# aweisberg/cassandra-accord

Measured on AMD Instinct MI355X. Metric: txn-key conflict pairs resolved/sec (node), higher is better.
Workload: dtype u32/u64 (integer); 1 GPU; config2: KeyDeps batch, 1M txns x 8 keys, zipf(0.99) over 1M keys, p_write 0.5, uncommitted window 10k, per-GPU CommandStore snapshot; key_distribution=zipf, keys_permuted=True, n_txn_per_gpu=1000000, pairs_per_gpu=8000000, dep_edges_per_gpu=35349420, parallelism=keyspace shards x1 (independent CommandStores)

## Files before the change

### cassandra-accord_amd/accord_amd/_lib.py

```python
from __future__ import annotations

import ctypes as C
import os

HERE = os.path.dirname(os.path.abspath(__file__))
LIB_PATH = os.environ.get("ACC_LIB_PATH") or os.path.join(HERE, "libaccord_amd.so")

ACC_OK, ACC_E_ARG, ACC_E_STATE, ACC_E_NOMEM, ACC_E_DEVICE, ACC_E_CAP = 0, -1, -2, -3, -4, -5
ACC_MEM_HOST, ACC_MEM_DEVICE = 0, 1
ACC_OPT_TIMING = 1
ACC_OPT_FORCE_REPLAY = 2
ACC_OPT_NO_WINDOW_TIER = 4
ACC_OPT_TIER_GRID_SHIFT = 16
ACC_OPT_RD_WIDE_SORT = 8
ACC_OPT_PD_SERIAL = 16
ACC_OPT_KD_NO_STREAM_AHEAD = 32
ACC_LV_AUTO, ACC_LV_LDS_WALK, ACC_LV_WINDOWED, ACC_LV_WAVES = 0, 1, 2, 3
ACC_STARTED_BEFORE, ACC_STARTED_AFTER, ACC_STARTED_ANY = 0, 1, 2
ACC_DEP_WITH, ACC_DEP_WITHOUT, ACC_DEP_ANY = 0, 1, 2
ACC_STATUS_ANY, ACC_STATUS_IS_PROPOSED, ACC_STATUS_IS_STABLE = 0, 1, 2
ACC_FULL_EXECUTES_AFTER = 1
ACC_LATEST_PROPOSAL, ACC_LATEST_COMMIT = 0, 1
RECOVERY_SCANS = {
    "acceptedOrCommittedStartedBeforeWithoutWitnessing": (ACC_STARTED_BEFORE, ACC_DEP_WITHOUT, ACC_STATUS_IS_PROPOSED, True),
# ... 11 lines not shown
           "acc_keydeps_batch", "acc_keydeps_copy_out", "acc_keydeps_mixed", "acc_rangedeps_batch", "acc_rangedeps_copy_out",
           "acc_shard_pack", "acc_shard_merge", "acc_keydeps_merge", "acc_merge_copy_out", "acc_levelise",
           "acc_timing_count", "acc_timing_get", "acc_timing_reset", "acc_timing_filter", "acc_stats_count", "acc_stats_get",
           "acc_deps_merge", "acc_rmm_copy_out", "acc_rmm_invert", "acc_rmm_slice", "acc_rangedeps_stab", "acc_copy_out", "acc_comm_unique_id", "acc_comm_init_rccl", "acc_comm_init_host", "acc_comm_destroy", "acc_partial_deps_reduce", "acc_shard_reduce",
           "acc_map_reduce_full", "acc_map_reduce_full_ranges", "acc_latest_deps_merge", "acc_partial_deps_batch",
           "acc_deps_from_json", "acc_deps_to_json",
           "acc_cfk_create", "acc_cfk_destroy", "acc_cfk_update", "acc_cfk_view", "acc_cfk_apply", "acc_cfk_snap_to_batch",
           "acc_cfk_apply_deps", "acc_cfk_state", "acc_cfk_missing", "acc_cfk_keydeps", "acc_cfk_keydeps_mixed",
           "acc_cfk_map_reduce_full", "acc_cfk_redundant_before", "acc_cfk_redundant_view", "acc_max_conflicts",
           "acc_maxconflicts_create", "acc_maxconflicts_destroy", "acc_maxconflicts_update", "acc_maxconflicts_get",
           "acc_maxconflicts_size",
           "acc_rcmd_create", "acc_rcmd_destroy", "acc_rcmd_update", "acc_rcmd_view", "acc_rcmd_rangedeps",
           "acc_rcmd_update_cmds", "acc_rcmd_state_view", "acc_rcmd_map_reduce_full",
           "acc_ranges_of", "acc_ranges_with", "acc_ranges_subtract", "acc_ranges_merge_touching", "acc_ranges_select",
           "acc_ranges_index_of", "acc_ranges_contains_all_keys", "acc_ranges_contains_all", "acc_rangedeps_is_covered_by",
           "acc_partial_deps_covering", "acc_rmm_without", "acc_recovery_deps_reduce"]


class Opts(C.Structure):
    _fields_ = [("flags", C.c_uint32), ("wave_grid_max", C.c_uint32), ("cfk_hot", C.c_uint32), ("lv_tier", C.c_uint32),
                ("lv_chunk", C.c_uint32), ("cfq_wave_cap", C.c_uint32)]


class TsCols(C.Structure):
    _fields_ = [("msb", C.c_void_p), ("lsb", C.c_void_p), ("node", C.c_void_p)]


class BatchIn(C.Structure):
    _fields_ = [("n_txn", C.c_uint32), ("mem", C.c_uint32), ("n_pairs", C.c_uint64),
                ("txn_id", TsCols), ("execute_at", TsCols),
                ("status", C.c_void_p), ("key_off", C.c_void_p), ("key_code", C.c_void_p)]
# ... 501 lines not shown
        L.acc_rcmd_view.argtypes = [C.c_void_p, C.c_void_p, C.POINTER(RcmdTable)]
        L.acc_rcmd_view.restype = C.c_int
        L.acc_rcmd_rangedeps.argtypes = [C.c_void_p, C.c_void_p, C.POINTER(CfkMixedQueries), C.POINTER(RangedepsView)]
        L.acc_rcmd_rangedeps.restype = C.c_int
        L.acc_rcmd_update_cmds.argtypes = [C.c_void_p, C.c_void_p, C.POINTER(RcmdCmdUpdates)]
        L.acc_rcmd_update_cmds.restype = C.c_int
        L.acc_rcmd_state_view.argtypes = [C.c_void_p, C.c_void_p, C.POINTER(RcmdState)]
        L.acc_rcmd_state_view.restype = C.c_int
        L.acc_rcmd_map_reduce_full.argtypes = [C.c_void_p, C.c_void_p, C.POINTER(CfkRecoveryIn), C.POINTER(RangedepsView)]
        L.acc_rcmd_map_reduce_full.restype = C.c_int
    except AttributeError:
        if not os.environ.get("ACC_LIB_PATH"):
            raise
    L.acc_copy_out.argtypes = [C.c_void_p, C.c_void_p, C.c_void_p, C.c_size_t, C.c_uint32]
    L.acc_copy_out.restype = C.c_int
    L.acc_timing_count.argtypes = [C.c_void_p]
    L.acc_timing_count.restype = C.c_int
    L.acc_timing_get.argtypes = [C.c_void_p, C.c_int, C.POINTER(C.c_char_p), C.POINTER(C.c_double),
                                 C.POINTER(C.c_uint64)]
    L.acc_timing_get.restype = C.c_int
    L.acc_timing_reset.argtypes = [C.c_void_p]
    L.acc_timing_reset.restype = None
    L.acc_timing_filter.argtypes = [C.c_void_p, C.c_char_p]
    L.acc_timing_filter.restype = C.c_int
    L.acc_stats_count.argtypes = [C.c_void_p]
    L.acc_stats_count.restype = C.c_int
    L.acc_stats_get.argtypes = [C.c_void_p, C.c_int, C.POINTER(C.c_char_p), C.POINTER(C.c_uint64)]
    L.acc_stats_get.restype = C.c_int
    _lib = L
    return L
# ... 1 lines not shown
```

### cassandra-accord_amd/accord_amd/deps.py

```python
from __future__ import annotations

import ctypes as C
from dataclasses import dataclass

import numpy as np

from . import _lib as L


class AccordError(RuntimeError):
    code = None


class IllegalArgumentException(AccordError):
    code = L.ACC_E_ARG


class IllegalStateException(AccordError):
    code = L.ACC_E_STATE


class DeviceError(AccordError):
    code = L.ACC_E_DEVICE

# ... 82 lines not shown

    def stats(self) -> dict:
        out = {}
        for i in range(max(self._lib.acc_stats_count(self._h), 0)):
            name = C.c_char_p()
            val = C.c_uint64()
            self._lib.acc_stats_get(self._h, i, C.byref(name), C.byref(val))
            out[name.value.decode()] = val.value
        return out

    def timing_reset(self):
        self._lib.acc_timing_reset(self._h)

    def timing_filter(self, tags=None):
        self.check(self._lib.acc_timing_filter(self._h, ",".join(tags).encode() if tags else None))

    def keydeps_batch_raw(self, batch_in: "L.BatchIn") -> "L.KeydepsView":
        view = L.KeydepsView()
        self.check(self._lib.acc_keydeps_batch(self._h, C.byref(batch_in), C.byref(view)))
        return view

    def calculate_partial_deps(self, batch) -> "BatchKeyDeps":
        arrs = dict(tm=np.ascontiguousarray(batch.txn_msb, dtype=np.uint64),
                    tl=np.ascontiguousarray(batch.txn_lsb, dtype=np.uint64),
                    tn=np.ascontiguousarray(batch.txn_node, dtype=np.int32),
                    em=np.ascontiguousarray(batch.exe_msb, dtype=np.uint64),
                    el=np.ascontiguousarray(batch.exe_lsb, dtype=np.uint64),
                    en=np.ascontiguousarray(batch.exe_node, dtype=np.int32),
                    st=np.ascontiguousarray(batch.status, dtype=np.uint8),
                    ko=np.ascontiguousarray(batch.key_off, dtype=np.uint32),
# ... 1146 lines not shown
```

### cassandra-accord_amd/csrc/api.hip

```cpp
#include "dict.hpp"
#include <exception>
#include <thread>

namespace acc {
void keydeps_batch(acc_ctx *ctx, const acc_batch_in *in, acc_keydeps_view *view);
void keydeps_mixed(acc_ctx *ctx, const acc_range_batch_in *in, acc_keydeps_view *view, SharedDict *shared = nullptr);
void keydeps_merge(acc_ctx *ctx, const acc_merge_in *in, acc_merge_view *view);
void levelise(acc_ctx *ctx, const acc_graph_in *in, uint32_t *level, uint32_t *order, uint32_t *n_levels);
void rangedeps_batch(acc_ctx *ctx, const acc_range_batch_in *in, acc_rangedeps_view *view, const SharedDict *shared = nullptr);
void shard_pack(acc_ctx *ctx, const acc_batch_in *in, acc_frag_streams *out, bool ctx_alloc);
void shard_merge(acc_ctx *ctx, const acc_frag_recv *in, acc_merge_view *view);
void deps_merge(acc_ctx *ctx, const acc_deps_merge_in *in, acc_deps_merge_view *view);
void rmm_invert(acc_ctx *ctx, const acc_rmm_batch *in, acc_csr_view *out);
void rmm_slice(acc_ctx *ctx, const acc_rmm_batch *in, const acc_ranges_in *select, acc_slice_view *out);
void rangedeps_stab(acc_ctx *ctx, const acc_rmm_batch *rd, const acc_stab_in *q, acc_stab_view *out);
void rmm_without(acc_ctx *ctx, const acc_rmm_batch *in, const acc_ts_cols *txn, const acc_txn_sets *set_a,
                 const acc_txn_sets *set_b, acc_without_view *out);
void recovery_deps_reduce(acc_ctx *ctx, const acc_deps_merge_in *cw, const acc_deps_merge_in *anw, acc_recovery_deps_view *view);
void map_reduce_full(acc_ctx *ctx, const acc_batch_in *in, const acc_recovery_in *q, acc_keydeps_view *view);
void map_reduce_full_ranges(acc_ctx *ctx, const acc_range_cmds_in *c, const acc_recovery_ranges_in *q, acc_rangedeps_view *view);
void latest_deps_merge(acc_ctx *ctx, const acc_latest_in *in, acc_latest_view *view);
void deps_from_json(acc_ctx *ctx, const acc_json_in *in, acc_json_deps_view *view);
void deps_to_json(acc_ctx *ctx, const acc_json_out_in *in, acc_json_out *out);
void cfk_update(acc_ctx *ctx, acc_cfk *cfk, const acc_batch_in *in);
// ... 93 lines not shown
}

}

extern "C" {

const char *acc_last_error(const acc_ctx *ctx) { return ctx ? ctx->last_error.c_str() : "null context"; }

int acc_sync(acc_ctx *ctx)
{
    if (!ctx) return ACC_E_ARG;
    return acc_guard(ctx, [&] { ctx->sync(); });
}

void *acc_stream(acc_ctx *ctx) { return ctx ? (void *)ctx->stream : nullptr; }

int acc_keydeps_batch(acc_ctx *ctx, const acc_batch_in *in, acc_keydeps_view *out_view)
{
    if (!ctx) return ACC_E_ARG;
    return acc_guard(ctx, [&] {
        ACC_HIP(hipSetDevice(ctx->device));
        acc::keydeps_batch(ctx, in, out_view);
    });
}

int acc_keydeps_mixed(acc_ctx *ctx, const acc_range_batch_in *in, acc_keydeps_view *out_view)
{
    if (!ctx) return ACC_E_ARG;
    return acc_guard(ctx, [&] {
        ACC_HIP(hipSetDevice(ctx->device));
// ... 612 lines not shown
```

### cassandra-accord_amd/csrc/keydeps.hip

```cpp
#include "keydeps.hpp"

#include <vector>

namespace acc {


struct TxnInfoArgs {
    uint32_t n = 0;
    const uint8_t *status = nullptr;
    const uint64_t *tl = nullptr;
    uint4 *tinfo = nullptr;
    uint32_t *bigflag = nullptr;
};

__device__ __forceinline__ void txn_info_one(uint32_t t, uint32_t n, const uint32_t *rank, const uint8_t *status,
                                             const uint64_t *tl, const uint32_t *key_off, uint4 *tinfo, uint32_t *bigflag)
{
    if (bigflag) bigflag[t] = 0;
    const uint32_t kind = (uint32_t)(tl[t] >> 1) & 7u;
    tinfo[t] = make_uint4(rank[t], rank[n + t], (uint32_t)status[t] | (kind << 3), key_off[t]);
}

__global__ __launch_bounds__(BLOCK) void k_pair_keys(size_t P, const uint64_t *__restrict__ key_code,
                                                     const uint32_t *__restrict__ owner, const uint32_t *__restrict__ key_off,
// ... 1 lines not shown
                                                     const uint32_t *__restrict__ perm, PairPlan plan,
                                                     int rank_only, uint64_t *__restrict__ out, TxnInfoArgs ti)
{
    size_t i = (size_t)blockIdx.x * BLOCK + threadIdx.x;
    if (ti.tinfo && i < ti.n) txn_info_one((uint32_t)i, ti.n, rank, ti.status, ti.tl, key_off, ti.tinfo, ti.bigflag);
    if (i >= P) return;
    size_t j = perm ? perm[i] : i;
    if (rank_only) { out[i] = rank[owner[j]]; return; }
    uint64_t kc = pext_runs(key_code[j], plan.rk);
    if (plan.mode == 4) {
        const uint32_t t = owner[j];
        out[i] = (kc << 32) | ((uint64_t)t << plan.sb) | (uint64_t)(j - key_off[t]);
        return;
    }
    out[i] = plan.mode == 1 ? ((kc << plan.rbits) | rank[owner[j]]) : plan.mode == 3 ? ((kc << 32) | i) : kc;
}

__global__ __launch_bounds__(BLOCK) void k_seg_flags_packed(size_t P, const uint64_t *__restrict__ sp, uint32_t *__restrict__ flag,
                                                            uint32_t *__restrict__ perm, int sb, const uint32_t *__restrict__ key_off,
                                                            uint32_t *__restrict__ pown)
{
    size_t p = (size_t)blockIdx.x * BLOCK + threadIdx.x;
    if (p >= P) return;
    const uint64_t x = sp[p];
    flag[p] = p == 0 || (x >> 32) != (sp[p - 1] >> 32);
    if (sb < 0) { perm[p] = (uint32_t)x; return; }
    const uint32_t t = (uint32_t)x >> sb, slot = (uint32_t)x & ((1u << sb) - 1u);
    perm[p] = key_off[t] + slot;
    pown[p] = t;
}
// ... 2413 lines not shown
    const size_t P = cb.P;
    const uint32_t *key_off = cb.key_off;
    const uint64_t *key_code = cb.key_code;
    const uint32_t *owner = cb.owner, *rank = cb.dict.rank;
    const int rbits = cb.dict.rbits;
    PairPlan &pp = cb.pp;
    uint64_t *pkey = ctx->get<uint64_t>("pair_key", P);
    const unsigned gP = grid_for(P, BLOCK);
    PairSort s;
    s.seg_flag = ctx->get<uint32_t>("seg_flag", P);
    if (cb.dict.batch_sorted && pp.rk.bits <= 32) {
        const bool m4 = bits_for((uint64_t)n - 1) + pp.sb <= 32;
        pp.mode = m4 ? 4 : 3;
        TxnInfoArgs ti;
        if (!keys_only) { ti.n = n; ti.status = cb.status; ti.tl = cb.tl; ti.tinfo = cb.tinfo; ti.bigflag = cb.bigflag; }
        launch(ctx, "pair_keys", k_pair_keys, dim3(grid_for(std::max<size_t>(P, n), BLOCK)), dim3(BLOCK), 0, P, key_code,
               owner, key_off, rank, (const uint32_t *)nullptr, pp, 0, pkey, ti);
        s.tinfo_done = !keys_only;
        const uint64_t *sp = radix_sort_keys(ctx, "rs_pair", pkey, P, 32, pp.rk.bits);
        uint32_t *perm = ctx->get<uint32_t>("pair_perm", P + V2_ITEMS);
        if (m4) s.sp_m4 = sp;
        else launch(ctx, "seg_flags", k_seg_flags_packed, dim3(gP), dim3(BLOCK), 0, P, sp, s.seg_flag, perm, -1, key_off,
                    (uint32_t *)nullptr);
        s.ps = { nullptr, perm };
        s.flags_done = true;
    } else if (cb.dict.batch_sorted) {
        pp.mode = 0;
        launch(ctx, "pair_keys", k_pair_keys, dim3(gP), dim3(BLOCK), 0, P, key_code, owner, key_off, rank,
               (const uint32_t *)nullptr, pp, 0, pkey, TxnInfoArgs{});
        s.ps = radix_sort(ctx, "rs_pair", pkey, nullptr, P, pp.rk.bits);
    } else if (pp.rk.bits + rbits <= 64) {
        pp.mode = 1;
        launch(ctx, "pair_keys", k_pair_keys, dim3(gP), dim3(BLOCK), 0, P, key_code, owner, key_off, rank,
               (const uint32_t *)nullptr, pp, 0, pkey, TxnInfoArgs{});
// ... 579 lines not shown
```

### cassandra-accord_amd/csrc/prims.hpp

```cpp
#pragma once

#include "ctx.hpp"

#include <algorithm>
#include <vector>

namespace acc {


__device__ __forceinline__ uint32_t lane_id() { return threadIdx.x & 63u; }

template <class T>
__device__ __forceinline__ T shfl_up(T v, unsigned d)
{
    if constexpr (sizeof(T) == 8) {
        uint64_t u = (uint64_t)v;
        uint32_t lo = __shfl_up((uint32_t)u, d, 64), hi = __shfl_up((uint32_t)(u >> 32), d, 64);
        return (T)(((uint64_t)hi << 32) | lo);
    } else {
        return (T)__shfl_up((uint32_t)v, d, 64);
    }
}

template <class T>
// ... 393 lines not shown

__device__ __forceinline__ uint64_t pext_runs(uint64_t w, const Runs &r)
{
    uint64_t o = 0;
    for (int i = 0; i < r.n; ++i) {
        uint64_t m = r.len[i] >= 64 ? ~0ull : ((1ull << r.len[i]) - 1);
        o |= ((w >> r.lo[i]) & m) << r.dst[i];
    }
    return o;
}


constexpr int RS_ITEMS = 16;
constexpr int RS_TILE = BLOCK * RS_ITEMS;
constexpr int RS_ITEMS_S = 4;
constexpr int RS_TILE_S = BLOCK * RS_ITEMS_S;
constexpr size_t rs_small_n() { return (size_t)256 << 10; }

static __global__ __launch_bounds__(BLOCK) void k_rs_hist(const uint64_t *__restrict__ keys, size_t n, int shift,
                                                   uint32_t *__restrict__ hist, uint32_t ntiles)
{
    __shared__ uint32_t h[256];
    h[threadIdx.x] = 0;
    __syncthreads();
    const size_t base = (size_t)blockIdx.x * RS_TILE;
#pragma unroll 4
    for (int k = 0; k < RS_ITEMS; ++k) {
        size_t e = base + (size_t)k * BLOCK + threadIdx.x;
        if (e < n) atomicAdd(&h[(keys[e] >> shift) & 255u], 1u);
    }
// ... 84 lines not shown
        }
    }
    __syncthreads();
    for (uint32_t i = tid; i < tile_total; i += BLOCK) {
        const uint64_t key = sk[i];
        const uint32_t d = (uint32_t)(key >> shift) & 255u;
        const uint32_t dst = gbase[d] + (i - lbase[d]);
        kout[dst] = key;
        vout[dst] = sv[i];
    }
}

constexpr uint32_t OS_AGG = 1u << 30, OS_INC = 2u << 30, OS_VAL = (1u << 30) - 1;
constexpr int OS_MAXP = 8;

static __global__ __launch_bounds__(BLOCK) void k_rs_ghist(const uint64_t *__restrict__ keys, size_t n, int lo, int passes,
                                                    uint32_t *__restrict__ ghist, uint32_t *__restrict__ other, uint32_t other_n)
{
    __shared__ uint32_t h[WAVES][OS_MAXP][256];
    const uint32_t tid = threadIdx.x, wave = tid >> 6, lane = lane_id();
    for (uint32_t i = blockIdx.x * BLOCK + tid; i < other_n; i += gridDim.x * BLOCK) other[i] = 0;
    for (uint32_t i = tid; i < WAVES * OS_MAXP * 256; i += BLOCK) (&h[0][0][0])[i] = 0;
    __syncthreads();
    for (size_t base = (size_t)blockIdx.x * RS_TILE; base < n; base += (size_t)gridDim.x * RS_TILE) {
    uint64_t key[RS_ITEMS];
#pragma unroll
    for (int k = 0; k < RS_ITEMS; ++k) {
        const size_t e = base + (size_t)k * BLOCK + tid;
        key[k] = e < n ? keys[e] : 0;
    }
    for (int p = 0; p < passes; ++p) {
#pragma unroll
        for (int k = 0; k < RS_ITEMS; ++k) {
            const bool valid = base + (size_t)k * BLOCK + tid < n;
            const uint32_t d = (uint32_t)(key[k] >> (lo + 8 * p)) & 255u;
            const uint32_t d0 = (uint32_t)__shfl((int)d, 0, 64);
            const uint64_t vb = __ballot(valid);
            if (__ballot(valid && d == d0) == vb) {
                if (lane == 0) h[wave][p][d0] += (uint32_t)__popcll(vb);
            } else if (valid) {
                atomicAdd(&h[wave][p][d], 1u);
            }
        }
    }
    }
    __syncthreads();
    for (uint32_t i = tid; i < (uint32_t)passes * 256; i += BLOCK) {
        uint32_t s = 0;
#pragma unroll
        for (int w = 0; w < WAVES; ++w) s += h[w][i >> 8][i & 255];
        if (s) atomicAdd(&ghist[i], s);
    }
}

__device__ __forceinline__ void os_store(uint32_t *p, uint32_t w) { __hip_atomic_store(p, w, __ATOMIC_RELAXED, __HIP_MEMORY_SCOPE_AGENT); }
__device__ __forceinline__ uint32_t os_load(const uint32_t *p) { return __hip_atomic_load(p, __ATOMIC_RELAXED, __HIP_MEMORY_SCOPE_AGENT); }

template <bool KO, int ITEMS>
static __global__ __launch_bounds__(BLOCK) void k_rs_onesweep(const uint64_t *__restrict__ kin, const uint32_t *__restrict__ vin,
                                                       uint64_t *__restrict__ kout, uint32_t *__restrict__ vout, size_t n,
                                                       int shift, const uint32_t *__restrict__ dtotal,
                                                       uint32_t *__restrict__ status, uint32_t *__restrict__ ticket,
                                                       int iota_vals)
{
    __shared__ uint64_t sk[(BLOCK * ITEMS)];
    __shared__ uint32_t sv[KO ? 1 : (BLOCK * ITEMS)];
    __shared__ uint32_t cnt[WAVES][256];
    __shared__ uint32_t wpre[WAVES][256];
    __shared__ uint32_t run[256], lbase[256], gbase[256];
    __shared__ uint32_t red[WAVES];
    __shared__ uint32_t s_b;
    const uint32_t tid = threadIdx.x, lane = lane_id(), wave = tid >> 6;
    const uint64_t lt_mask = (lane == 0) ? 0ull : ((~0ull) >> (64 - lane));
    if (tid == 0) s_b = atomicAdd(ticket, 1u);
    run[tid] = 0;
#pragma unroll
    for (int w = 0; w < WAVES; ++w) cnt[w][tid] = 0;
    __syncthreads();
    const uint32_t b = s_b;
    const size_t base = (size_t)b * (BLOCK * ITEMS);
    uint64_t key[ITEMS];
    uint32_t val[ITEMS], lr[ITEMS], pk[ITEMS];
#pragma unroll
    for (int k = 0; k < ITEMS; ++k) {
        const size_t e = base + (size_t)k * BLOCK + tid;
        const bool valid = e < n;
        key[k] = valid ? kin[e] : 0;
        if constexpr (!KO) val[k] = valid ? (iota_vals ? (uint32_t)e : vin[e]) : 0;
    }
#pragma unroll
    for (int k = 0; k < ITEMS; ++k) {
        const bool valid = base + (size_t)k * BLOCK + tid < n;
        const uint32_t d = (uint32_t)(key[k] >> shift) & 255u;
        uint64_t peers = __ballot(valid);
#pragma unroll
        for (int bb = 0; bb < 8; ++bb) {
            const uint64_t bal = __ballot((d >> bb) & 1u);
            peers &= ((d >> bb) & 1u) ? bal : ~bal;
        }
        const uint32_t rank = (uint32_t)__popcll(peers & lt_mask);
        pk[k] = rank | ((uint32_t)__popcll(peers) << 16);
        if (valid && rank == 0) atomicAdd(&run[d], (uint32_t)__popcll(peers));
    }
    __syncthreads();
    const uint32_t c = run[tid];
    uint32_t *st = status + (size_t)b * 256;
    os_store(&st[tid], b == 0 ? (c | OS_INC) : (c | OS_AGG));
    uint32_t tile_total;
    const uint32_t lb = block_exclusive(c, OpAdd<uint32_t>(), red, tile_total);
    run[tid] = 0;
    lbase[tid] = lb;
    __syncthreads();
#pragma unroll
    for (int k = 0; k < ITEMS; ++k) {
        const bool valid = base + (size_t)k * BLOCK + tid < n;
        const uint32_t d = (uint32_t)(key[k] >> shift) & 255u;
        const uint32_t rank = pk[k] & 0xFFFFu;
        if (valid && rank == 0) cnt[wave][d] = pk[k] >> 16;
        __syncthreads();
        {
            uint32_t r = run[tid];
#pragma unroll
            for (int w = 0; w < WAVES; ++w) {
                wpre[w][tid] = r;
                r += cnt[w][tid];
                cnt[w][tid] = 0;
            }
            run[tid] = r;
        }
        __syncthreads();
        lr[k] = wpre[wave][d] + rank;
    }
#pragma unroll
    for (int k = 0; k < ITEMS; ++k) {
        const size_t e = base + (size_t)k * BLOCK + tid;
        if (e < n) {
            const uint32_t d = (uint32_t)(key[k] >> shift) & 255u;
            const uint32_t dst = lbase[d] + lr[k];
            sk[dst] = key[k];
            if constexpr (!KO) sv[dst] = val[k];
        }
    }
    uint32_t all;
    const uint32_t dbase = block_exclusive(dtotal[tid], OpAdd<uint32_t>(), red, all);
    uint32_t pre = 0;
    if (b > 0) {
#ifndef ACC_OS_LB
#define ACC_OS_LB 8
#endif
        constexpr int LB = ACC_OS_LB;
        for (int64_t j = (int64_t)b - 1;; j -= LB) {
            uint32_t w[LB];
#pragma unroll
            for (int u = 0; u < LB; ++u) w[u] = j - u >= 0 ? os_load(&status[(size_t)(j - u) * 256 + tid]) : OS_INC;
            bool done = false;
#pragma unroll
            for (int u = 0; u < LB; ++u) {
                if (done) continue;
                while ((w[u] >> 30) == 0) {
                    __builtin_amdgcn_s_sleep(1);
                    w[u] = os_load(&status[(size_t)(j - u) * 256 + tid]);
                }
                pre += w[u] & OS_VAL;
                done = (w[u] >> 30) == 2;
            }
            if (done) break;
        }
        os_store(&st[tid], (pre + c) | OS_INC);
    }
    gbase[tid] = dbase + pre;
    __syncthreads();
    for (uint32_t i = tid; i < tile_total; i += BLOCK) {
        const uint64_t k2 = sk[i];
        const uint32_t d = (uint32_t)(k2 >> shift) & 255u;
        const uint32_t dst = gbase[d] + (i - lbase[d]);
        kout[dst] = k2;
        if constexpr (!KO) vout[dst] = sv[i];
    }
}

static __global__ void k_iota(uint32_t *__restrict__ out, size_t n)
{
    size_t i = (size_t)blockIdx.x * blockDim.x + threadIdx.x;
    if (i < n) out[i] = (uint32_t)i;
}

[[maybe_unused]] static __global__ __launch_bounds__(BLOCK) void k_widen_u32(size_t n, const uint32_t *__restrict__ in, uint64_t *__restrict__ out)
{
    const size_t p = (size_t)blockIdx.x * BLOCK + threadIdx.x;
    if (p < n) out[p] = in[p];
}

[[maybe_unused]] static __global__ __launch_bounds__(BLOCK) void k_permute_u64(size_t n, const uint32_t *__restrict__ perm,
                                                              const uint64_t *__restrict__ in, uint64_t *__restrict__ out)
{
    const size_t p = (size_t)blockIdx.x * BLOCK + threadIdx.x;
    if (p < n) out[p] = in[perm[p]];
}

struct Sorted {
    uint64_t *keys;
    uint32_t *vals;
};

struct OsWords {
    uint32_t *cur, *other;
    uint32_t other_n;
    acc_ctx::OsState *st;
    size_t words;
    void commit() const
    {
        st->dirty[st->par] = words;
        st->dirty[st->par ^ 1] = 0;
// ... 30 lines not shown
    int passes = (bits + 7) / 8;
    if (n == 0) return { k[0], v[0] };
    if (passes == 0) {
        ACC_HIP(hipMemcpyAsync(k[0], keys, n * sizeof(uint64_t), hipMemcpyDeviceToDevice, ctx->cur()));
        if (vals) ACC_HIP(hipMemcpyAsync(v[0], vals, n * sizeof(uint32_t), hipMemcpyDeviceToDevice, ctx->cur()));
        else launch(ctx, "iota", k_iota, dim3(grid_for(n, BLOCK)), dim3(BLOCK), 0, v[0], n);
        return { k[0], v[0] };
    }
    if (n < (size_t)OS_VAL && passes <= OS_MAXP) {
        const bool small = n < rs_small_n();
        const uint32_t ntiles = (uint32_t)((n + (small ? RS_TILE_S : RS_TILE) - 1) / (small ? RS_TILE_S : RS_TILE));
        const size_t words = (size_t)passes * 256 + passes + (size_t)passes * ntiles * 256;
        const OsWords ow = os_words(ctx, tag, words);
        uint32_t *ghist = ow.cur, *tickets = ow.cur + (size_t)passes * 256, *status = tickets + passes;
        snprintf(th, sizeof th, "%s.ghist", tag);
        launch(ctx, th, k_rs_ghist, dim3(std::min<unsigned>(ntiles, 1024u)), dim3(BLOCK), 0, keys, n, 0, passes, ghist, ow.other,
               ow.other_n);
        ow.commit();
        const uint64_t *kin = keys;
        const uint32_t *vin = vals;
        int cur = 0;
        for (int p = 0; p < passes; ++p) {
            if (small)
                launch(ctx, ts, k_rs_onesweep<false, RS_ITEMS_S>, dim3(ntiles), dim3(BLOCK), 0, kin, vin, k[cur], v[cur], n, 8 * p,
                       (const uint32_t *)(ghist + (size_t)p * 256), status + (size_t)p * ntiles * 256, tickets + p,
                       (p == 0 && !vals) ? 1 : 0);
            else
                launch(ctx, ts, k_rs_onesweep<false, RS_ITEMS>, dim3(ntiles), dim3(BLOCK), 0, kin, vin, k[cur], v[cur], n, 8 * p,
                       (const uint32_t *)(ghist + (size_t)p * 256), status + (size_t)p * ntiles * 256, tickets + p,
                       (p == 0 && !vals) ? 1 : 0);
            kin = k[cur];
            vin = v[cur];
// ... 10 lines not shown
    const uint32_t *vin = vals;
    int cur = 0;
    for (int p = 0; p < passes; ++p) {
        int shift = 8 * p;
        launch(ctx, th, k_rs_hist, dim3(ntiles), dim3(BLOCK), 0, kin, n, shift, hist, ntiles);
        launch(ctx, "rs_colscan", k_rs_colscan, dim3(256), dim3(BLOCK), 0, hist, ntiles, dtot);
        launch(ctx, ts, k_rs_scatter, dim3(ntiles), dim3(BLOCK), 0, kin, vin, k[cur], v[cur], n, shift,
               (const uint32_t *)hist, (const uint32_t *)dtot, ntiles, (p == 0 && !vals) ? 1 : 0);
        kin = k[cur];
        vin = v[cur];
        cur ^= 1;
    }
    return { (uint64_t *)kin, (uint32_t *)vin };
}

static inline uint64_t *radix_sort_keys(acc_ctx *ctx, const char *tag, const uint64_t *keys, size_t n, int lo, int bits)
{
    char nk0[40], nk1[40], th[48], ts[48];
    snprintf(nk0, sizeof nk0, "%s_k0", tag); snprintf(nk1, sizeof nk1, "%s_k1", tag);
    snprintf(th, sizeof th, "%s.ghist", tag);
    snprintf(ts, sizeof ts, "%s.scatter", tag);
    uint64_t *k[2] = { ctx->get<uint64_t>(nk0, n), ctx->get<uint64_t>(nk1, n) };
    const int passes = (bits + 7) / 8;
    if (n >= (size_t)OS_VAL || passes > OS_MAXP) fail(ACC_E_CAP, "internal: keys-only radix sort beyond its limits");
    if (n == 0 || passes == 0) {
        if (n) ACC_HIP(hipMemcpyAsync(k[0], keys, n * sizeof(uint64_t), hipMemcpyDeviceToDevice, ctx->cur()));
        return k[0];
    }
    const bool small = n < rs_small_n();
    const uint32_t ntiles = (uint32_t)((n + (small ? RS_TILE_S : RS_TILE) - 1) / (small ? RS_TILE_S : RS_TILE));
    const size_t words = (size_t)passes * 256 + passes + (size_t)passes * ntiles * 256;
    const OsWords ow = os_words(ctx, tag, words);
    uint32_t *ghist = ow.cur, *tickets = ow.cur + (size_t)passes * 256, *status = tickets + passes;
    launch(ctx, th, k_rs_ghist, dim3(std::min<unsigned>(ntiles, 1024u)), dim3(BLOCK), 0, keys, n, lo, passes, ghist, ow.other,
           ow.other_n);
    ow.commit();
    const uint64_t *kin = keys;
    int cur = 0;
    for (int p = 0; p < passes; ++p) {
        if (small)
            launch(ctx, ts, k_rs_onesweep<true, RS_ITEMS_S>, dim3(ntiles), dim3(BLOCK), 0, kin, (const uint32_t *)nullptr, k[cur],
                   (uint32_t *)nullptr, n, lo + 8 * p, (const uint32_t *)(ghist + (size_t)p * 256),
                   status + (size_t)p * ntiles * 256, tickets + p, 0);
        else
            launch(ctx, ts, k_rs_onesweep<true, RS_ITEMS>, dim3(ntiles), dim3(BLOCK), 0, kin, (const uint32_t *)nullptr, k[cur],
                   (uint32_t *)nullptr, n, lo + 8 * p, (const uint32_t *)(ghist + (size_t)p * 256),
                   status + (size_t)p * ntiles * 256, tickets + p, 0);
        kin = k[cur];
        cur ^= 1;
    }
    return (uint64_t *)kin;
}

inline int bits_for(uint64_t max_value)
{
    return max_value == 0 ? 0 : 64 - __builtin_clzll(max_value);
}

#ifdef ACC_PHASE_PROF
template <class Sym>
inline unsigned long long *prof_arm(acc_ctx *ctx, const char *name, const Sym &symbol, size_t words, hipStream_t st)
{
    unsigned long long *buf = ctx->get<unsigned long long>(name, words);
    ACC_HIP(hipMemsetAsync(buf, 0, words * sizeof(unsigned long long), st));
    ACC_HIP(hipMemcpyToSymbolAsync(symbol, &buf, sizeof buf, 0, hipMemcpyHostToDevice, st));
    return buf;
}
inline std::vector<unsigned long long> prof_read(const unsigned long long *buf, size_t words, hipStream_t st)
{
    std::vector<unsigned long long> h(words);
    ACC_HIP(hipMemcpyAsync(h.data(), buf, words * sizeof(unsigned long long), hipMemcpyDeviceToHost, st));
    ACC_HIP(hipStreamSynchronize(st));
    return h;
}
#endif

}
```

### include/accord_amd.h

```cpp
#ifndef ACCORD_AMD_H
#define ACCORD_AMD_H

#include <stdint.h>
#include <stddef.h>

#ifdef __cplusplus
extern "C" {
#endif

typedef struct acc_rlist {
    const uint64_t *start;
    const uint64_t *end;
    uint32_t n;
    uint32_t reserved;
} acc_rlist;

#define ACC_OK          0
#define ACC_E_ARG      (-1)
#define ACC_E_STATE    (-2)
#define ACC_E_NOMEM    (-3)
#define ACC_E_DEVICE   (-4)
#define ACC_E_CAP      (-5)

#define ACC_ST_TRANSITIVELY_KNOWN   0
// ... 709 lines not shown
                      uint32_t cap, uint32_t *out_n);
int acc_ranges_index_of(const acc_rlist *a, uint32_t end_inclusive, uint64_t key, int64_t *out_index);
int acc_ranges_contains_all_keys(const acc_rlist *a, uint32_t end_inclusive, const uint64_t *keys, uint32_t n_keys,
                                 int32_t *out);
int acc_ranges_contains_all(const acc_rlist *a, const acc_rlist *b, int32_t *out);
int acc_rangedeps_is_covered_by(const acc_rlist *range_deps_ranges, const acc_rlist *covering, int32_t *out);

int  acc_timing_count(acc_ctx *ctx);
int  acc_timing_get(acc_ctx *ctx, int i, const char **name, double *total_ms, uint64_t *launches);
void acc_timing_reset(acc_ctx *ctx);
int  acc_timing_filter(acc_ctx *ctx, const char *tags_csv);

int acc_stats_count(acc_ctx *ctx);
int acc_stats_get(acc_ctx *ctx, int i, const char **name, uint64_t *value);

#ifdef __cplusplus
}
#endif
#endif
```

Baseline: 3.901 billion txn-key pairs/s.

## Fuse radix histogram into pair-key kernel and streamline onesweep ranking

Computes the radix-sort global digit histogram inside the pair-key generation kernel, so the separate ghist pass that re-reads all pair keys is no longer needed. It also rewrites the onesweep ranking to use per-wave running counts in LDS with wave-contiguous loads, replacing the per-item block barriers and extra prefix arrays. The scatter step gets simpler index arithmetic. It adds a diagnostic sort API and optional phase profiling, and the wave-local non-atomic LDS update relies on wave barriers for correctness.

```diff
diff --git a/cassandra-accord_amd/accord_amd/_lib.py b/cassandra-accord_amd/accord_amd/_lib.py
--- a/cassandra-accord_amd/accord_amd/_lib.py
+++ b/cassandra-accord_amd/accord_amd/_lib.py
@@ -49,7 +49,7 @@
            "acc_rcmd_update_cmds", "acc_rcmd_state_view", "acc_rcmd_map_reduce_full",
            "acc_ranges_of", "acc_ranges_with", "acc_ranges_subtract", "acc_ranges_merge_touching", "acc_ranges_select",
            "acc_ranges_index_of", "acc_ranges_contains_all_keys", "acc_ranges_contains_all", "acc_rangedeps_is_covered_by",
-           "acc_partial_deps_covering", "acc_rmm_without", "acc_recovery_deps_reduce"]
+           "acc_partial_deps_covering", "acc_rmm_without", "acc_recovery_deps_reduce", "acc_sort_u64"]
 
 
 class Opts(C.Structure):
@@ -581,6 +581,9 @@
             raise
     L.acc_copy_out.argtypes = [C.c_void_p, C.c_void_p, C.c_void_p, C.c_size_t, C.c_uint32]
     L.acc_copy_out.restype = C.c_int
+    L.acc_sort_u64.argtypes = [C.c_void_p, C.c_void_p, C.c_void_p, C.c_uint64, C.c_int, C.c_int, C.c_int, C.c_void_p,
+                               C.c_void_p]
+    L.acc_sort_u64.restype = C.c_int
     L.acc_timing_count.argtypes = [C.c_void_p]
     L.acc_timing_count.restype = C.c_int
     L.acc_timing_get.argtypes = [C.c_void_p, C.c_int, C.POINTER(C.c_char_p), C.POINTER(C.c_double),
diff --git a/cassandra-accord_amd/accord_amd/deps.py b/cassandra-accord_amd/accord_amd/deps.py
--- a/cassandra-accord_amd/accord_amd/deps.py
+++ b/cassandra-accord_amd/accord_amd/deps.py
@@ -120,6 +120,11 @@
 
     def timing_filter(self, tags=None):
         self.check(self._lib.acc_timing_filter(self._h, ",".join(tags).encode() if tags else None))
+
+    def sort_u64(self, keys, vals, n: int, lo: int, bits: int, keys_only: bool, out_keys, out_vals=None):
+        p = lambda t: C.c_void_p(t.data_ptr() or None) if t is not None else None
+        self.check(self._lib.acc_sort_u64(self._h, p(keys), p(vals), int(n), int(lo), int(bits), int(bool(keys_only)),
+                                          p(out_keys), p(out_vals)))
 
     def keydeps_batch_raw(self, batch_in: "L.BatchIn") -> "L.KeydepsView":
         view = L.KeydepsView()
diff --git a/cassandra-accord_amd/csrc/api.hip b/cassandra-accord_amd/csrc/api.hip
--- a/cassandra-accord_amd/csrc/api.hip
+++ b/cassandra-accord_amd/csrc/api.hip
@@ -131,6 +131,28 @@
 }
 
 void *acc_stream(acc_ctx *ctx) { return ctx ? (void *)ctx->stream : nullptr; }
+
+int acc_sort_u64(acc_ctx *ctx, const uint64_t *keys, const uint32_t *vals, uint64_t n, int lo, int bits, int keys_only,
+                 uint64_t *out_keys, uint32_t *out_vals)
+{
+    if (!ctx) return ACC_E_ARG;
+    return acc_guard(ctx, [&] {
+        ACC_HIP(hipSetDevice(ctx->device));
+        if (lo < 0 || bits < 0 || lo + bits > 64 || (!keys_only && lo != 0)) acc::fail(ACC_E_ARG, "acc_sort_u64: bad bit range");
+        if (n && (!keys || !out_keys || (!keys_only && !out_vals))) acc::fail(ACC_E_ARG, "null argument");
+        if (keys_only) {
+            const uint64_t *sk = acc::radix_sort_keys(ctx, "diag_sort", keys, (size_t)n, lo, bits);
+            if (n) ACC_HIP(hipMemcpyAsync(out_keys, sk, n * sizeof(uint64_t), hipMemcpyDeviceToDevice, ctx->cur()));
+        } else {
+            const acc::Sorted s = acc::radix_sort(ctx, "diag_sort", keys, vals, (size_t)n, bits);
+            if (n) {
+                ACC_HIP(hipMemcpyAsync(out_keys, s.keys, n * sizeof(uint64_t), hipMemcpyDeviceToDevice, ctx->cur()));
+                ACC_HIP(hipMemcpyAsync(out_vals, s.vals, n * sizeof(uint32_t), hipMemcpyDeviceToDevice, ctx->cur()));
+            }
+        }
+        ctx->sync();
+    });
+}
 
 int acc_keydeps_batch(acc_ctx *ctx, const acc_batch_in *in, acc_keydeps_view *out_view)
 {
diff --git a/cassandra-accord_amd/csrc/keydeps.hip b/cassandra-accord_amd/csrc/keydeps.hip
--- a/cassandra-accord_amd/csrc/keydeps.hip
+++ b/cassandra-accord_amd/csrc/keydeps.hip
@@ -39,6 +39,26 @@
         return;
     }
     out[i] = plan.mode == 1 ? ((kc << plan.rbits) | rank[owner[j]]) : plan.mode == 3 ? ((kc << 32) | i) : kc;
+}
+
+__global__ __launch_bounds__(BLOCK) void k_pair_keys_hist(size_t P, const uint64_t *__restrict__ key_code,
+                                                          const uint32_t *__restrict__ owner, const uint32_t *__restrict__ key_off,
+                                                          const uint32_t *__restrict__ rank, PairPlan plan,
+                                                          uint64_t *__restrict__ out, TxnInfoArgs ti, OsHist hist)
+{
+    if (ti.tinfo)
+        for (size_t t = (size_t)blockIdx.x * BLOCK + threadIdx.x; t < ti.n; t += (size_t)gridDim.x * BLOCK)
+            txn_info_one((uint32_t)t, ti.n, rank, ti.status, ti.tl, key_off, ti.tinfo, ti.bigflag);
+    os_hist_block(P, hist, [&](size_t i) {
+        const uint64_t kc = pext_runs(key_code[i], plan.rk);
+        uint64_t x = (kc << 32) | i;
+        if (plan.mode == 4) {
+            const uint32_t t = owner[i];
+            x = (kc << 32) | ((uint64_t)t << plan.sb) | (uint64_t)(i - key_off[t]);
+        }
+        out[i] = x;
+        return x;
+    });
 }
 
 __global__ __launch_bounds__(BLOCK) void k_seg_flags_packed(size_t P, const uint64_t *__restrict__ sp, uint32_t *__restrict__ flag,
@@ -2482,10 +2502,11 @@
         pp.mode = m4 ? 4 : 3;
         TxnInfoArgs ti;
         if (!keys_only) { ti.n = n; ti.status = cb.status; ti.tl = cb.tl; ti.tinfo = cb.tinfo; ti.bigflag = cb.bigflag; }
-        launch(ctx, "pair_keys", k_pair_keys, dim3(grid_for(std::max<size_t>(P, n), BLOCK)), dim3(BLOCK), 0, P, key_code,
-               owner, key_off, rank, (const uint32_t *)nullptr, pp, 0, pkey, ti);
+        const KeySortPlan pl = radix_sort_keys_prepare(ctx, "rs_pair", P, 32, pp.rk.bits);
+        launch(ctx, "pair_keys", k_pair_keys_hist, dim3(std::max(1u, os_hist_grid(P))), dim3(BLOCK), 0, P, key_code, owner,
+               key_off, rank, pp, pkey, ti, pl.hist);
         s.tinfo_done = !keys_only;
-        const uint64_t *sp = radix_sort_keys(ctx, "rs_pair", pkey, P, 32, pp.rk.bits);
+        const uint64_t *sp = radix_sort_keys_sort(ctx, "rs_pair", pl, pkey);
         uint32_t *perm = ctx->get<uint32_t>("pair_perm", P + V2_ITEMS);
         if (m4) s.sp_m4 = sp;
         else launch(ctx, "seg_flags", k_seg_flags_packed, dim3(gP), dim3(BLOCK), 0, P, sp, s.seg_flag, perm, -1, key_off,
diff --git a/cassandra-accord_amd/csrc/prims.hpp b/cassandra-accord_amd/csrc/prims.hpp
--- a/cassandra-accord_amd/csrc/prims.hpp
+++ b/cassandra-accord_amd/csrc/prims.hpp
@@ -431,6 +431,11 @@
 constexpr int RS_ITEMS = 16;
 constexpr int RS_TILE = BLOCK * RS_ITEMS;
 constexpr int RS_ITEMS_S = 4;
+#ifndef ACC_RS_ITEMS_KO
+#define ACC_RS_ITEMS_KO 16
+#endif
+constexpr int RS_ITEMS_KO = ACC_RS_ITEMS_KO;
+constexpr int RS_TILE_KO = BLOCK * RS_ITEMS_KO;
 constexpr int RS_TILE_S = BLOCK * RS_ITEMS_S;
 constexpr size_t rs_small_n() { return (size_t)256 << 10; }
 
@@ -545,47 +550,66 @@
 constexpr uint32_t OS_AGG = 1u << 30, OS_INC = 2u << 30, OS_VAL = (1u << 30) - 1;
 constexpr int OS_MAXP = 8;
 
-static __global__ __launch_bounds__(BLOCK) void k_rs_ghist(const uint64_t *__restrict__ keys, size_t n, int lo, int passes,
-                                                    uint32_t *__restrict__ ghist, uint32_t *__restrict__ other, uint32_t other_n)
+struct OsHist {
+    uint32_t *ghist = nullptr, *other = nullptr;
+    uint32_t other_n = 0;
+    int lo = 0, passes = 0;
+};
+
+template <class KeyAt>
+__device__ __forceinline__ void os_hist_block(size_t n, const OsHist &a, KeyAt key_at)
 {
     __shared__ uint32_t h[WAVES][OS_MAXP][256];
     const uint32_t tid = threadIdx.x, wave = tid >> 6, lane = lane_id();
-    for (uint32_t i = blockIdx.x * BLOCK + tid; i < other_n; i += gridDim.x * BLOCK) other[i] = 0;
+    for (uint32_t i = blockIdx.x * BLOCK + tid; i < a.other_n; i += gridDim.x * BLOCK) a.other[i] = 0;
     for (uint32_t i = tid; i < WAVES * OS_MAXP * 256; i += BLOCK) (&h[0][0][0])[i] = 0;
     __syncthreads();
     for (size_t base = (size_t)blockIdx.x * RS_TILE; base < n; base += (size_t)gridDim.x * RS_TILE) {
-    uint64_t key[RS_ITEMS];
-#pragma unroll
-    for (int k = 0; k < RS_ITEMS; ++k) {
-        const size_t e = base + (size_t)k * BLOCK + tid;
-        key[k] = e < n ? keys[e] : 0;
-    }
-    for (int p = 0; p < passes; ++p) {
+        uint64_t key[RS_ITEMS];
 #pragma unroll
         for (int k = 0; k < RS_ITEMS; ++k) {
-            const bool valid = base + (size_t)k * BLOCK + tid < n;
-            const uint32_t d = (uint32_t)(key[k] >> (lo + 8 * p)) & 255u;
-            const uint32_t d0 = (uint32_t)__shfl((int)d, 0, 64);
-            const uint64_t vb = __ballot(valid);
-            if (__ballot(valid && d == d0) == vb) {
-                if (lane == 0) h[wave][p][d0] += (uint32_t)__popcll(vb);
-            } else if (valid) {
-                atomicAdd(&h[wave][p][d], 1u);
+            const size_t e = base + (size_t)k * BLOCK + tid;
+            key[k] = e < n ? key_at(e) : 0;
+        }
+        for (int p = 0; p < a.passes; ++p) {
+#pragma unroll
+            for (int k = 0; k < RS_ITEMS; ++k) {
+                const bool valid = base + (size_t)k * BLOCK + tid < n;
+                const uint32_t d = (uint32_t)(key[k] >> (a.lo + 8 * p)) & 255u;
+                const uint32_t d0 = (uint32_t)__shfl((int)d, 0, 64);
+                const uint64_t vb = __ballot(valid);
+                if (__ballot(valid && d == d0) == vb) {
+                    if (lane == 0) h[wave][p][d0] += (uint32_t)__popcll(vb);
+                } else if (valid) {
+                    atomicAdd(&h[wave][p][d], 1u);
+                }
             }
         }
     }
-    }
-    __syncthreads();
-    for (uint32_t i = tid; i < (uint32_t)passes * 256; i += BLOCK) {
+    __syncthreads();
+    for (uint32_t i = tid; i < (uint32_t)a.passes * 256; i += BLOCK) {
         uint32_t s = 0;
 #pragma unroll
         for (int w = 0; w < WAVES; ++w) s += h[w][i >> 8][i & 255];
-        if (s) atomicAdd(&ghist[i], s);
-    }
+        if (s) atomicAdd(&a.ghist[i], s);
+    }
+}
+inline unsigned os_hist_grid(size_t n) { return (unsigned)std::min<size_t>((n + RS_TILE - 1) / RS_TILE, 1024); }
+
+static __global__ __launch_bounds__(BLOCK) void k_rs_ghist(const uint64_t *__restrict__ keys, size_t n, OsHist a)
+{
+    os_hist_block(n, a, [&](size_t e) { return keys[e]; });
 }
 
 __device__ __forceinline__ void os_store(uint32_t *p, uint32_t w) { __hip_atomic_store(p, w, __ATOMIC_RELAXED, __HIP_MEMORY_SCOPE_AGENT); }
 __device__ __forceinline__ uint32_t os_load(const uint32_t *p) { return __hip_atomic_load(p, __ATOMIC_RELAXED, __HIP_MEMORY_SCOPE_AGENT); }
+
+#ifdef ACC_PHASE_PROF
+static __device__ unsigned long long *g_rs_prof;
+#define RS_PH(i) rs_ph[i] = clock64()
+#else
+#define RS_PH(i) ((void)0)
+#endif
 
 template <bool KO, int ITEMS>
 static __global__ __launch_bounds__(BLOCK) void k_rs_onesweep(const uint64_t *__restrict__ kin, const uint32_t *__restrict__ vin,
@@ -597,31 +621,39 @@
     __shared__ uint64_t sk[(BLOCK * ITEMS)];
     __shared__ uint32_t sv[KO ? 1 : (BLOCK * ITEMS)];
     __shared__ uint32_t cnt[WAVES][256];
-    __shared__ uint32_t wpre[WAVES][256];
-    __shared__ uint32_t run[256], lbase[256], gbase[256];
+    __shared__ uint32_t gbase[256];
     __shared__ uint32_t red[WAVES];
     __shared__ uint32_t s_b;
     const uint32_t tid = threadIdx.x, lane = lane_id(), wave = tid >> 6;
     const uint64_t lt_mask = (lane == 0) ? 0ull : ((~0ull) >> (64 - lane));
+#ifdef ACC_PHASE_PROF
+    unsigned long long rs_ph[7];
+#endif
+    RS_PH(0);
     if (tid == 0) s_b = atomicAdd(ticket, 1u);
-    run[tid] = 0;
 #pragma unroll
     for (int w = 0; w < WAVES; ++w) cnt[w][tid] = 0;
+    const uint32_t dt = dtotal[tid];
     __syncthreads();
     const uint32_t b = s_b;
-    const size_t base = (size_t)b * (BLOCK * ITEMS);
+    const size_t base = (size_t)b * (BLOCK * ITEMS) + (size_t)wave * (64 * ITEMS) + lane;
     uint64_t key[ITEMS];
-    uint32_t val[ITEMS], lr[ITEMS], pk[ITEMS];
+    uint32_t val[ITEMS], lr[ITEMS];
 #pragma unroll
     for (int k = 0; k < ITEMS; ++k) {
-        const size_t e = base + (size_t)k * BLOCK + tid;
+        const size_t e = base + (size_t)k * 64;
         const bool valid = e < n;
         key[k] = valid ? kin[e] : 0;
         if constexpr (!KO) val[k] = valid ? (iota_vals ? (uint32_t)e : vin[e]) : 0;
     }
+#ifdef ACC_PHASE_PROF
+    asm volatile("s_waitcnt vmcnt(0)" ::: "memory");
+#endif
+    RS_PH(1);
+    uint32_t *wc = cnt[wave];
 #pragma unroll
     for (int k = 0; k < ITEMS; ++k) {
-        const bool valid = base + (size_t)k * BLOCK + tid < n;
+        const bool valid = base + (size_t)k * 64 < n;
         const uint32_t d = (uint32_t)(key[k] >> shift) & 255u;
         uint64_t peers = __ballot(valid);
 #pragma unroll
@@ -630,50 +662,38 @@
             peers &= ((d >> bb) & 1u) ? bal : ~bal;
         }
         const uint32_t rank = (uint32_t)__popcll(peers & lt_mask);
-        pk[k] = rank | ((uint32_t)__popcll(peers) << 16);
-        if (valid && rank == 0) atomicAdd(&run[d], (uint32_t)__popcll(peers));
-    }
-    __syncthreads();
-    const uint32_t c = run[tid];
+        const uint32_t before = wc[d];
+        lr[k] = before + rank;
+        __builtin_amdgcn_wave_barrier();
+        if (valid && rank == 0) wc[d] = before + (uint32_t)__popcll(peers);
+        __builtin_amdgcn_wave_barrier();
+        __builtin_amdgcn_fence(__ATOMIC_RELEASE, "wavefront");
+    }
+    __syncthreads();
+    RS_PH(2);
+    uint32_t wp[WAVES], c = 0;
+#pragma unroll
+    for (int w = 0; w < WAVES; ++w) { wp[w] = c; c += cnt[w][tid]; }
     uint32_t *st = status + (size_t)b * 256;
     os_store(&st[tid], b == 0 ? (c | OS_INC) : (c | OS_AGG));
     uint32_t tile_total;
     const uint32_t lb = block_exclusive(c, OpAdd<uint32_t>(), red, tile_total);
-    run[tid] = 0;
-    lbase[tid] = lb;
-    __syncthreads();
+#pragma unroll
+    for (int w = 0; w < WAVES; ++w) cnt[w][tid] = lb + wp[w];
+    __syncthreads();
+    RS_PH(3);
 #pragma unroll
     for (int k = 0; k < ITEMS; ++k) {
-        const bool valid = base + (size_t)k * BLOCK + tid < n;
-        const uint32_t d = (uint32_t)(key[k] >> shift) & 255u;
-        const uint32_t rank = pk[k] & 0xFFFFu;
-        if (valid && rank == 0) cnt[wave][d] = pk[k] >> 16;
-        __syncthreads();
-        {
-            uint32_t r = run[tid];
-#pragma unroll
-            for (int w = 0; w < WAVES; ++w) {
-                wpre[w][tid] = r;
-                r += cnt[w][tid];
-                cnt[w][tid] = 0;
-            }
-            run[tid] = r;
-        }
-        __syncthreads();
-        lr[k] = wpre[wave][d] + rank;
-    }
-#pragma unroll
-    for (int k = 0; k < ITEMS; ++k) {
-        const size_t e = base + (size_t)k * BLOCK + tid;
-        if (e < n) {
+        if (base + (size_t)k * 64 < n) {
             const uint32_t d = (uint32_t)(key[k] >> shift) & 255u;
-            const uint32_t dst = lbase[d] + lr[k];
+            const uint32_t dst = wc[d] + lr[k];
             sk[dst] = key[k];
             if constexpr (!KO) sv[dst] = val[k];
         }
     }
     uint32_t all;
-    const uint32_t dbase = block_exclusive(dtotal[tid], OpAdd<uint32_t>(), red, all);
+    const uint32_t dbase = block_exclusive(dt, OpAdd<uint32_t>(), red, all);
+    RS_PH(4);
     uint32_t pre = 0;
     if (b > 0) {
 #ifndef ACC_OS_LB
@@ -699,15 +719,23 @@
         }
         os_store(&st[tid], (pre + c) | OS_INC);
     }
-    gbase[tid] = dbase + pre;
-    __syncthreads();
+    gbase[tid] = dbase + pre - lb;
+    __syncthreads();
+    RS_PH(5);
     for (uint32_t i = tid; i < tile_total; i += BLOCK) {
         const uint64_t k2 = sk[i];
-        const uint32_t d = (uint32_t)(k2 >> shift) & 255u;
-        const uint32_t dst = gbase[d] + (i - lbase[d]);
+        const uint32_t dst = gbase[(uint32_t)(k2 >> shift) & 255u] + i;
         kout[dst] = k2;
         if constexpr (!KO) vout[dst] = sv[i];
     }
+#ifdef ACC_PHASE_PROF
+    RS_PH(6);
+    if (tid == 0 && g_rs_prof) {
+        unsigned long long *row = g_rs_prof + (size_t)b * 8;
+        for (int i = 0; i < 6; ++i) row[i] = rs_ph[i + 1] - rs_ph[i];
+        row[7] = 1;
+    }
+#endif
 }
 
 static __global__ void k_iota(uint32_t *__restrict__ out, size_t n)
@@ -728,6 +756,24 @@
     const size_t p = (size_t)blockIdx.x * BLOCK + threadIdx.x;
     if (p < n) out[p] = in[perm[p]];
 }
+
+#ifdef ACC_PHASE_PROF
+template <class Sym>
+inline unsigned long long *prof_arm(acc_ctx *ctx, const char *name, const Sym &symbol, size_t words, hipStream_t st)
+{
+    unsigned long long *buf = ctx->get<unsigned long long>(name, words);
+    ACC_HIP(hipMemsetAsync(buf, 0, words * sizeof(unsigned long long), st));
+    ACC_HIP(hipMemcpyToSymbolAsync(symbol, &buf, sizeof buf, 0, hipMemcpyHostToDevice, st));
+    return buf;
+}
+inline std::vector<unsigned long long> prof_read(const unsigned long long *buf, size_t words, hipStream_t st)
+{
+    std::vector<unsigned long long> h(words);
+    ACC_HIP(hipMemcpyAsync(h.data(), buf, words * sizeof(unsigned long long), hipMemcpyDeviceToHost, st));
+    ACC_HIP(hipStreamSynchronize(st));
+    return h;
+}
+#endif
 
 struct Sorted {
     uint64_t *keys;
@@ -788,8 +834,7 @@
         const OsWords ow = os_words(ctx, tag, words);
         uint32_t *ghist = ow.cur, *tickets = ow.cur + (size_t)passes * 256, *status = tickets + passes;
         snprintf(th, sizeof th, "%s.ghist", tag);
-        launch(ctx, th, k_rs_ghist, dim3(std::min<unsigned>(ntiles, 1024u)), dim3(BLOCK), 0, keys, n, 0, passes, ghist, ow.other,
-               ow.other_n);
+        launch(ctx, th, k_rs_ghist, dim3(os_hist_grid(n)), dim3(BLOCK), 0, keys, n, OsHist{ ghist, ow.other, ow.other_n, 0, passes });
         ow.commit();
         const uint64_t *kin = keys;
         const uint32_t *vin = vals;
@@ -830,65 +875,99 @@
     return { (uint64_t *)kin, (uint32_t *)vin };
 }
 
-static inline uint64_t *radix_sort_keys(acc_ctx *ctx, const char *tag, const uint64_t *keys, size_t n, int lo, int bits)
-{
-    char nk0[40], nk1[40], th[48], ts[48];
+struct KeySortPlan {
+    OsHist hist;
+    uint64_t *k[2] = { nullptr, nullptr };
+    uint32_t *tickets = nullptr, *status = nullptr;
+    size_t n = 0;
+    int lo = 0, passes = 0;
+    uint32_t ntiles = 0;
+    bool small = false;
+};
+static inline KeySortPlan radix_sort_keys_prepare(acc_ctx *ctx, const char *tag, size_t n, int lo, int bits)
+{
+    char nk0[40], nk1[40];
     snprintf(nk0, sizeof nk0, "%s_k0", tag); snprintf(nk1, sizeof nk1, "%s_k1", tag);
-    snprintf(th, sizeof th, "%s.ghist", tag);
-    snprintf(ts, sizeof ts, "%s.scatter", tag);
-    uint64_t *k[2] = { ctx->get<uint64_t>(nk0, n), ctx->get<uint64_t>(nk1, n) };
+    KeySortPlan pl;
+    pl.k[0] = ctx->get<uint64_t>(nk0, n); pl.k[1] = ctx->get<uint64_t>(nk1, n);
+    pl.n = n; pl.lo = lo;
     const int passes = (bits + 7) / 8;
     if (n >= (size_t)OS_VAL || passes > OS_MAXP) fail(ACC_E_CAP, "internal: keys-only radix sort beyond its limits");
-    if (n == 0 || passes == 0) {
-        if (n) ACC_HIP(hipMemcpyAsync(k[0], keys, n * sizeof(uint64_t), hipMemcpyDeviceToDevice, ctx->cur()));
-        return k[0];
-    }
-    const bool small = n < rs_small_n();
-    const uint32_t ntiles = (uint32_t)((n + (small ? RS_TILE_S : RS_TILE) - 1) / (small ? RS_TILE_S : RS_TILE));
-    const size_t words = (size_t)passes * 256 + passes + (size_t)passes * ntiles * 256;
+    if (n == 0 || passes == 0) return pl;
+    pl.passes = passes;
+    pl.small = n < rs_small_n();
+    pl.ntiles = (uint32_t)((n + (pl.small ? RS_TILE_S : RS_TILE_KO) - 1) / (pl.small ? RS_TILE_S : RS_TILE_KO));
+    const size_t words = (size_t)passes * 256 + passes + (size_t)passes * pl.ntiles * 256;
     const OsWords ow = os_words(ctx, tag, words);
-    uint32_t *ghist = ow.cur, *tickets = ow.cur + (size_t)passes * 256, *status = tickets + passes;
-    launch(ctx, th, k_rs_ghist, dim3(std::min<unsigned>(ntiles, 1024u)), dim3(BLOCK), 0, keys, n, lo, passes, ghist, ow.other,
-           ow.other_n);
+    pl.tickets = ow.cur + (size_t)passes * 256;
+    pl.status = pl.tickets + passes;
+    pl.hist = OsHist{ ow.cur, ow.other, ow.other_n, lo, passes };
     ow.commit();
+    return pl;
+}
+static inline uint64_t *radix_sort_keys_sort(acc_ctx *ctx, const char *tag, const KeySortPlan &pl, const uint64_t *keys)
+{
+    char ts[48];
+    snprintf(ts, sizeof ts, "%s.scatter", tag);
+    const size_t n = pl.n;
+    if (pl.passes == 0) {
+        if (n) ACC_HIP(hipMemcpyAsync(pl.k[0], keys, n * sizeof(uint64_t), hipMemcpyDeviceToDevice, ctx->cur()));
+        return pl.k[0];
+    }
     const uint64_t *kin = keys;
     int cur = 0;
-    for (int p = 0; p < passes; ++p) {
-        if (small)
-            launch(ctx, ts, k_rs_onesweep<true, RS_ITEMS_S>, dim3(ntiles), dim3(BLOCK), 0, kin, (const uint32_t *)nullptr, k[cur],
-                   (uint32_t *)nullptr, n, lo + 8 * p, (const uint32_t *)(ghist + (size_t)p * 256),
-                   status + (size_t)p * ntiles * 256, tickets + p, 0);
+#ifdef ACC_PHASE_PROF
+    const bool prof = !strcmp(tag, "rs_pair") && !pl.small;
+#endif
+    for (int p = 0; p < pl.passes; ++p) {
+#ifdef ACC_PHASE_PROF
+        unsigned long long *prof_buf = prof ? prof_arm(ctx, "rs_prof", HIP_SYMBOL(g_rs_prof), 8 * (size_t)pl.ntiles, ctx->cur()) : nullptr;
+#endif
+        if (pl.small)
+            launch(ctx, ts, k_rs_onesweep<true, RS_ITEMS_S>, dim3(pl.ntiles), dim3(BLOCK), 0, kin, (const uint32_t *)nullptr,
+                   pl.k[cur], (uint32_t *)nullptr, n, pl.lo + 8 * p, (const uint32_t *)(pl.hist.ghist + (size_t)p * 256),
+                   pl.status + (size_t)p * pl.ntiles * 256, pl.tickets + p, 0);
         else
-            launch(ctx, ts, k_rs_onesweep<true, RS_ITEMS>, dim3(ntiles), dim3(BLOCK), 0, kin, (const uint32_t *)nullptr, k[cur],
-                   (uint32_t *)nullptr, n, lo + 8 * p, (const uint32_t *)(ghist + (size_t)p * 256),
-                   status + (size_t)p * ntiles * 256, tickets + p, 0);
-        kin = k[cur];
+            launch(ctx, ts, k_rs_onesweep<true, RS_ITEMS_KO>, dim3(pl.ntiles), dim3(BLOCK), 0, kin, (const uint32_t *)nullptr,
+                   pl.k[cur], (uint32_t *)nullptr, n, pl.lo + 8 * p, (const uint32_t *)(pl.hist.ghist + (size_t)p * 256),
+                   pl.status + (size_t)p * pl.ntiles * 256, pl.tickets + p, 0);
+#ifdef ACC_PHASE_PROF
+        if (prof) {
+            const std::vector<unsigned long long> h = prof_read(prof_buf, 8 * (size_t)pl.ntiles, ctx->cur());
+            unsigned long long *none = nullptr;
+            ACC_HIP(hipMemcpyToSymbolAsync(HIP_SYMBOL(g_rs_prof), &none, sizeof none, 0, hipMemcpyHostToDevice, ctx->cur()));
+            double sum[6] = {}, mx[6] = {};
+            size_t w = 0;
+            for (size_t r = 0; r < pl.ntiles; ++r) {
+                if (!h[8 * r + 7]) continue;
+                ++w;
+                for (int i = 0; i < 6; ++i) { sum[i] += (double)h[8 * r + i]; mx[i] = std::max(mx[i], (double)h[8 * r + i]); }
+            }
+            const double d = w ? (double)w : 1.0;
+            fprintf(stderr, "[rs_phase] pass=%d tiles=%zu avg cycles: load %.0f rank %.0f count+publish %.0f lds-reorder %.0f lookback %.0f scatter %.0f | max: %.0f %.0f %.0f %.0f %.0f %.0f\n",
+                    p, w, sum[0] / d, sum[1] / d, sum[2] / d, sum[3] / d, sum[4] / d, sum[5] / d, mx[0], mx[1], mx[2], mx[3], mx[4], mx[5]);
+        }
+#endif
+        kin = pl.k[cur];
         cur ^= 1;
     }
     return (uint64_t *)kin;
 }
+static inline uint64_t *radix_sort_keys(acc_ctx *ctx, const char *tag, const uint64_t *keys, size_t n, int lo, int bits)
+{
+    const KeySortPlan pl = radix_sort_keys_prepare(ctx, tag, n, lo, bits);
+    if (pl.passes) {
+        char th[48];
+        snprintf(th, sizeof th, "%s.ghist", tag);
+        launch(ctx, th, k_rs_ghist, dim3(os_hist_grid(n)), dim3(BLOCK), 0, keys, n, pl.hist);
+    }
+    return radix_sort_keys_sort(ctx, tag, pl, keys);
+}
 
 inline int bits_for(uint64_t max_value)
 {
     return max_value == 0 ? 0 : 64 - __builtin_clzll(max_value);
 }
 
-#ifdef ACC_PHASE_PROF
-template <class Sym>
-inline unsigned long long *prof_arm(acc_ctx *ctx, const char *name, const Sym &symbol, size_t words, hipStream_t st)
-{
-    unsigned long long *buf = ctx->get<unsigned long long>(name, words);
-    ACC_HIP(hipMemsetAsync(buf, 0, words * sizeof(unsigned long long), st));
-    ACC_HIP(hipMemcpyToSymbolAsync(symbol, &buf, sizeof buf, 0, hipMemcpyHostToDevice, st));
-    return buf;
-}
-inline std::vector<unsigned long long> prof_read(const unsigned long long *buf, size_t words, hipStream_t st)
-{
-    std::vector<unsigned long long> h(words);
-    ACC_HIP(hipMemcpyAsync(h.data(), buf, words * sizeof(unsigned long long), hipMemcpyDeviceToHost, st));
-    ACC_HIP(hipStreamSynchronize(st));
-    return h;
-}
-#endif
-
-}
+
+}
diff --git a/include/accord_amd.h b/include/accord_amd.h
--- a/include/accord_amd.h
+++ b/include/accord_amd.h
@@ -747,6 +747,9 @@
 int acc_stats_count(acc_ctx *ctx);
 int acc_stats_get(acc_ctx *ctx, int i, const char **name, uint64_t *value);
 
+int acc_sort_u64(acc_ctx *ctx, const uint64_t *keys, const uint32_t *vals, uint64_t n, int lo, int bits, int keys_only,
+                 uint64_t *out_keys, uint32_t *out_vals);
+
 #ifdef __cplusplus
 }
 #endif
```

Result: slower. 3.831 billion txn-key pairs/s (-1.8%).
